# TheJacksonLaboratory/cnn_autoencoder

Measured on AMD Instinct MI355X. Metric: tiles/sec, compress+decompress round trip of 1024x1024x3 histology tiles, higher is better.
Workload: dtype f32 (f16x3 split MFMA: 3 f16 MFMAs per product, fp32 accumulate)

## Files before the change

### cnn_autoencoder_amd/_lib.py

```python
from __future__ import annotations

import ctypes
import os
import subprocess
import threading

import torch

_HERE = os.path.dirname(os.path.abspath(__file__))
LIB_PATH = os.environ.get('CAE_LIB') or os.path.join(_HERE, 'libcae_hip.so')
_lock = threading.Lock()
_lib = None

c_void_p = ctypes.c_void_p
c_int = ctypes.c_int
c_size_t = ctypes.c_size_t
c_float = ctypes.c_float

SYMBOLS = {
    'cae_version': (c_int, []),
    'cae_last_error': (ctypes.c_char_p, []),
    'cae_free': (None, [c_void_p]),
    'cae_model_create': (c_int, [c_int, c_int, c_int, c_int, c_int, ctypes.POINTER(c_void_p)]),
    'cae_model_destroy': (None, [c_void_p]),
# ... 9 lines not shown
    'cae_analysis_levels': (c_int, [c_void_p, c_void_p, c_int, c_int, c_int, c_int, c_void_p, c_void_p, c_void_p]),
    'cae_synthesis': (c_int, [c_void_p, c_void_p, c_int, c_int, c_int, c_void_p, c_int, c_void_p, c_void_p]),
    'cae_model_set_layer_stage': (c_int, [c_void_p, c_int, c_int, c_int, c_void_p, c_void_p, c_void_p, c_void_p, c_int,
                                           c_int, c_int]),
    'cae_model_set_color_layer': (c_int, [c_void_p, c_int, c_int, c_int, c_void_p, c_void_p]),
    'cae_synthesis_multiscale': (c_int, [c_void_p, c_void_p, c_int, c_int, c_int, c_void_p, c_int, c_void_p, c_void_p,
                                          c_void_p]),
    'cae_analysis_symbols': (c_int, [c_void_p, c_void_p, c_int, c_int, c_int, c_int, c_void_p, c_void_p]),
    'cae_synthesis_symbols': (c_int, [c_void_p, c_void_p, c_int, c_int, c_int, c_void_p, c_int, c_void_p]),
    'cae_synthesis_scale': (c_int, [c_void_p, c_void_p, c_int, c_int, c_int, c_int, c_void_p, c_int, c_void_p]),
    'cae_synthesis_symbols_scale': (c_int, [c_void_p, c_void_p, c_int, c_int, c_int, c_int, c_void_p, c_int, c_void_p]),
    'cae_gdn_forward': (c_int, [c_void_p, c_int, c_int, c_void_p, c_int, c_int, c_int, c_void_p, c_void_p]),
    'cae_quantize': (c_int, [c_void_p, c_void_p, c_int, c_int, c_void_p, c_void_p]),
    'cae_quantize_export': (c_int, [c_void_p, c_void_p, c_int, c_int, c_void_p, c_int, c_void_p]),
    'cae_copy_to_host': (c_int, [c_void_p, c_void_p, c_size_t]),
    'cae_dequantize': (c_int, [c_void_p, c_void_p, c_int, c_int, c_void_p, c_void_p]),
    'cae_model_set_density': (c_int, [c_void_p, c_int, c_int, c_void_p, c_void_p, c_void_p, c_void_p, c_float]),
    'cae_model_set_likelihood_form': (c_int, [c_void_p, c_int]),
    'cae_likelihood': (c_int, [c_void_p, c_void_p, c_int, c_int, c_void_p, c_void_p, c_void_p, c_void_p]),
    'cae_tile_ssim': (c_int, [c_void_p, c_void_p, c_int, c_int, c_int, c_int, c_void_p, c_void_p, c_size_t, c_void_p]),
    'cae_tile_delta_e': (c_int, [c_void_p, c_void_p, c_int, c_size_t, c_void_p, c_void_p, c_size_t, c_void_p]),
    'cae_u8hwc_to_planes': (c_int, [c_void_p, c_int, c_int, c_int, c_int, c_void_p, c_void_p]),
    'cae_avgpool2': (c_int, [c_void_p, c_int, c_int, c_int, c_void_p, c_void_p]),
    'cae_msssim_level': (c_int, [c_void_p, c_void_p, c_int, c_int, c_int, c_void_p, c_void_p, c_void_p, c_size_t, c_void_p]),
    'cae_tile_sse': (c_int, [c_void_p, c_void_p, c_int, c_size_t, c_void_p, c_void_p]),
    'cae_model_set_profiling': (c_int, [c_void_p, c_int]),
    'cae_model_get_profile': (c_int, [c_void_p, c_int, c_void_p, c_int, c_void_p, c_int]),
    'cae_t_packed_bytes': (c_size_t, [c_int, c_int, c_int]),
    'cae_t_pack_weights': (c_int, [c_void_p, c_int, c_int, c_int, c_int, c_void_p, c_void_p]),
    'cae_t_from_nchw': (c_int, [c_void_p, c_int, c_int, c_int, c_int, c_int, c_void_p, c_void_p, c_void_p]),
# ... 57 lines not shown
                                     c_void_p, c_void_p]),
    'cae_t_sample_labeled_patches': (c_int, [c_void_p, c_void_p, c_int, c_int, c_int, c_int, c_int, c_void_p, c_void_p,
                                             c_void_p, c_void_p, c_void_p, c_void_p, c_void_p, ctypes.c_uint64,
                                             ctypes.c_uint32, c_float, c_int, c_int, c_int, c_int, c_void_p, c_size_t,
                                             c_void_p, c_void_p, c_void_p]),
    'cae_t_elastic_deform': (c_int, [c_void_p, c_void_p, c_void_p, c_int, c_int, c_int, c_int, c_void_p, c_size_t, c_void_p,
                                     c_void_p, c_void_p]),
    'cae_t_elastic_deform_workspace': (c_size_t, [c_int, c_int, c_int]),
    'cae_cpu_budget': (c_int, []),
    'cae_coder_lockstep': (c_int, []),
    'cae_coder_threads': (c_int, [c_int, c_int]),
    'cae_pmf_to_quantized_cdf': (c_int, [c_void_p, c_int, c_int, c_void_p]),
    'cae_rans_encode_batch': (c_int, [c_void_p, c_void_p, c_int, c_int, c_void_p, c_void_p, c_int]),
    'cae_rans_encode_packed': (c_int, [c_void_p, c_void_p, c_int, c_int, c_void_p, c_void_p, c_int]),
    'cae_rans_decode_batch': (c_int, [c_void_p, c_void_p, c_void_p, c_int, c_int, c_void_p, c_int]),
    'cae_rans_encode_workspace': (c_int, [c_void_p, c_int, c_int, ctypes.POINTER(c_size_t)]),
    'cae_rans_encode_device': (c_int, [c_void_p, c_void_p, c_int, c_int, c_void_p, c_size_t, c_void_p, c_void_p, c_void_p,
                                       c_size_t, c_void_p]),
    'cae_rans_decode_device': (c_int, [c_void_p, c_void_p, c_size_t, c_void_p, c_int, c_int, c_void_p, c_void_p, c_void_p]),
    'cae_door_create': (c_int, [c_void_p, c_void_p, c_int, c_int, ctypes.POINTER(c_void_p)]),
    'cae_door_destroy': (None, [c_void_p]),
    'cae_door_encode': (c_int, [c_void_p, c_void_p, c_int, c_int, c_int, ctypes.POINTER(c_void_p),
                                ctypes.POINTER(c_size_t)]),
    'cae_door_decode_shape': (c_int, [c_void_p, c_void_p, c_size_t, ctypes.POINTER(c_int), ctypes.POINTER(c_int),
                                      ctypes.POINTER(c_int)]),
    'cae_door_decode': (c_int, [c_void_p, c_void_p, c_size_t, c_void_p, c_size_t]),
    'cae_door_stats': (c_int, [c_void_p, c_void_p, c_int, c_int]),
    'cae_door_hold': (c_int, [c_void_p, c_int]),
    'cae_seg_plan': (c_int, [c_void_p, c_void_p, c_int]),
    'cae_seg_workspace_bytes': (c_int, [c_void_p, c_int, c_int, c_int, c_void_p]),
# ... 120 lines not shown
```

### cnn_autoencoder_amd/csrc/cae_copy.cpp

```cpp
#include "cae_hip.h"
#include "cae_internal.hpp"

#include <hsa/hsa.h>
#include <hsa/hsa_ext_amd.h>

#include <mutex>

using namespace cae;

extern "C" int cae_copy_to_host(void *dst_host, const void *src_dev, size_t bytes) {
    if (!dst_host || !src_dev) return fail(CAE_ERR_ARG, "NULL argument");
    if (bytes == 0) return CAE_OK;
    static std::once_flag once;
    static hsa_status_t init_status = HSA_STATUS_SUCCESS;
    std::call_once(once, [] { init_status = hsa_init(); });
    if (init_status != HSA_STATUS_SUCCESS) return fail(CAE_ERR_HIP, "hsa_init failed (%d)", (int)init_status);

    hsa_amd_pointer_info_t si{}, di{};
    si.size = sizeof(si);
    di.size = sizeof(di);
    hsa_status_t st = hsa_amd_pointer_info(const_cast<void *>(src_dev), &si, nullptr, nullptr, nullptr);
    if (st != HSA_STATUS_SUCCESS || si.type != HSA_EXT_POINTER_TYPE_HSA)
        return fail(CAE_ERR_ARG, "source is not a device allocation of this process");
    st = hsa_amd_pointer_info(dst_host, &di, nullptr, nullptr, nullptr);
    if (st != HSA_STATUS_SUCCESS || (di.type != HSA_EXT_POINTER_TYPE_HSA && di.type != HSA_EXT_POINTER_TYPE_LOCKED))
        return fail(CAE_ERR_ARG, "destination must be pinned host memory (hipHostMalloc / a pinned tensor)");
    const char *s0 = (const char *)si.agentBaseAddress, *d0 = (const char *)di.agentBaseAddress;
    if ((const char *)src_dev + bytes > s0 + si.sizeInBytes || (const char *)dst_host + bytes > d0 + di.sizeInBytes)
        return fail(CAE_ERR_ARG, "copy of %zu bytes leaves its allocation", bytes);

    hsa_signal_t sig;
    st = hsa_signal_create(1, 0, nullptr, &sig);
    if (st != HSA_STATUS_SUCCESS) return fail(CAE_ERR_HIP, "hsa_signal_create failed (%d)", (int)st);
    st = hsa_amd_memory_async_copy(dst_host, di.agentOwner, src_dev, si.agentOwner, bytes, 0, nullptr, sig);
    if (st != HSA_STATUS_SUCCESS) {
        hsa_signal_destroy(sig);
        return fail(CAE_ERR_HIP, "hsa_amd_memory_async_copy failed (%d)", (int)st);
    }
    while (hsa_signal_wait_scacquire(sig, HSA_SIGNAL_CONDITION_LT, 1, UINT64_MAX, HSA_WAIT_STATE_BLOCKED) >= 1) {
    }
    hsa_signal_destroy(sig);
    return CAE_OK;
}
```

### cnn_autoencoder_amd/csrc/cae_entropy.cpp

```cpp
#include "cae_hip.h"
#include "cae_internal.hpp"

#include <algorithm>
#include <atomic>
#include <cmath>
#include <cstdio>
#include <cstdlib>
#include <cstring>
#include <mutex>
#include <string>
#include <thread>

#include <sched.h>

namespace cae {

static constexpr uint64_t kRansL = 1ull << 31;
static constexpr uint32_t kPrecision = 16;
static constexpr uint32_t kBypassBits = 4;
static constexpr uint32_t kMaxBypass = (1u << kBypassBits) - 1;
#ifndef CAE_CODER_LOCKSTEP
#define CAE_CODER_LOCKSTEP 2
#endif
static constexpr int kLockMax = 4;
// ... 350 lines not shown
                }
            }
        }
    };
    if (threads == 1) {
        work();
    } else {
        std::vector<std::thread> pool;
        for (int t = 0; t < threads; ++t) pool.emplace_back(work);
        for (auto &t : pool) t.join();
    }
    if (rc.load() != 0) return fail(rc.load(), "%s", first_err.c_str());
    return CAE_OK;
}

}

int rans_encode_chunk(const EntropyTables &T, const int32_t *symbols, int hw, size_t headroom, uint8_t **out,
                      size_t *out_len) {
    const int32_t *sy[1] = {symbols};
    return encode_streams<1>(T, sy, hw, out, out_len, headroom);
}

int rans_encode_chunk_pair(const EntropyTables &T, const int32_t *const *symbols, int hw, size_t headroom, uint8_t **out,
                           size_t *out_len) {
    return encode_streams<2>(T, symbols, hw, out, out_len, headroom);
}

int rans_decode_chunk(const EntropyTables &T, const uint8_t *buf, size_t len, int hw, int32_t *symbols) {
    const uint8_t *b[1] = {buf};
// ... 67 lines not shown
int cae_rans_encode_batch(cae_model_t *mm, const int32_t *symbols, int n_streams, int hw, uint8_t **out_bufs,
                          size_t *out_lens, int threads) {
    Model *m = reinterpret_cast<Model *>(mm);
    if (!m || !symbols || !out_bufs || !out_lens) return fail(CAE_ERR_ARG, "NULL argument");
    if (m->ent.channels == 0) return fail(CAE_ERR_ARG, "entropy model not set");
    if (n_streams < 1 || hw < 0) return fail(CAE_ERR_ARG, "bad shape");
    for (int i = 0; i < n_streams; ++i) {
        out_bufs[i] = nullptr;
        out_lens[i] = 0;
    }
    const EntropyTables &T = m->ent;
    const size_t per = (size_t)T.channels * hw;
    const int lock = lockstep_width();
    const int items = (n_streams + lock - 1) / lock;
    int rc = parallel_streams(items, threads, [&](int it) {
        int i = lock * it;
        const int end = std::min(n_streams, i + lock);
        int r = CAE_OK;
        const int32_t *sy[kLockMax];
        for (; r == CAE_OK && i + 3 < end; i += 4) {
            for (int k = 0; k < 4; ++k) sy[k] = symbols + per * (i + k);
            r = encode_streams<4>(T, sy, hw, &out_bufs[i], &out_lens[i]);
        }
        for (; r == CAE_OK && i + 1 < end; i += 2) {
            sy[0] = symbols + per * i;
            sy[1] = symbols + per * (i + 1);
            r = encode_streams<2>(T, sy, hw, &out_bufs[i], &out_lens[i]);
        }
        if (r == CAE_OK && i < end) {
            sy[0] = symbols + per * i;
            r = encode_streams<1>(T, sy, hw, &out_bufs[i], &out_lens[i]);
        }
        return r;
    });
    if (rc != 0)
        for (int i = 0; i < n_streams; ++i) {
            free(out_bufs[i]);
            out_bufs[i] = nullptr;
        }
    return rc;
}

int cae_rans_encode_packed(cae_model_t *mm, const int32_t *symbols, int n_streams, int hw, uint8_t **out_buf,
                           size_t *offsets, int threads) {
    if (!out_buf || !offsets) return fail(CAE_ERR_ARG, "NULL argument");
    *out_buf = nullptr;
    std::vector<uint8_t *> bufs((size_t)std::max(n_streams, 1), nullptr);
    std::vector<size_t> lens((size_t)std::max(n_streams, 1), 0);
    int rc = cae_rans_encode_batch(mm, symbols, n_streams, hw, bufs.data(), lens.data(), threads);
    if (rc) return rc;
    offsets[0] = 0;
    for (int i = 0; i < n_streams; ++i) offsets[i + 1] = offsets[i] + lens[i];
    uint8_t *packed = (uint8_t *)malloc(offsets[n_streams] ? offsets[n_streams] : 1);
    if (!packed) rc = fail(CAE_ERR_NOMEM, "out of memory (%zu bytes)", offsets[n_streams]);
    if (rc == CAE_OK)
        rc = parallel_streams(n_streams, threads, [&](int i) {
            memcpy(packed + offsets[i], bufs[i], lens[i]);
            return (int)CAE_OK;
        });
    for (int i = 0; i < n_streams; ++i) free(bufs[i]);
    if (rc) {
        free(packed);
        return rc;
    }
    *out_buf = packed;
    return CAE_OK;
}

int cae_rans_decode_batch(cae_model_t *mm, const uint8_t *const *bufs, const size_t *lens, int n_streams, int hw,
                          int32_t *symbols, int threads) {
    Model *m = reinterpret_cast<Model *>(mm);
    if (!m || !symbols || !bufs || !lens) return fail(CAE_ERR_ARG, "NULL argument");
    if (m->ent.channels == 0) return fail(CAE_ERR_ARG, "entropy model not set");
    if (n_streams < 1 || hw < 0) return fail(CAE_ERR_ARG, "bad shape");
    const EntropyTables &T = m->ent;
    const size_t per = (size_t)T.channels * hw;
    const int lock = lockstep_width();
    const int items = (n_streams + lock - 1) / lock;
    return parallel_streams(items, threads, [&](int it) {
        int i = lock * it;
        const int end = std::min(n_streams, i + lock);
        int r = CAE_OK;
        int32_t *sy[kLockMax];
        for (; r == CAE_OK && i + 3 < end; i += 4) {
            for (int k = 0; k < 4; ++k) sy[k] = symbols + per * (i + k);
            r = decode_streams<4>(T, bufs + i, lens + i, hw, sy);
        }
        for (; r == CAE_OK && i + 1 < end; i += 2) {
            sy[0] = symbols + per * i;
            sy[1] = symbols + per * (i + 1);
            r = decode_streams<2>(T, bufs + i, lens + i, hw, sy);
        }
        if (r == CAE_OK && i < end) {
            sy[0] = symbols + per * i;
            r = decode_streams<1>(T, bufs + i, lens + i, hw, sy);
        }
        return r;
    });
}

}
```

### cnn_autoencoder_amd/csrc/cae_internal.hpp

```cpp
#pragma once
#include <cstdarg>
#include <cstddef>
#include <cstdint>
#include <mutex>
#include <utility>
#include <vector>

namespace cae {

int fail(int code, const char *fmt, ...);

void dev_free(void *p);

struct DevBuf {
    void *p = nullptr;
    size_t bytes = 0;
    DevBuf() = default;
    DevBuf(DevBuf &&o) noexcept : p(o.p), bytes(o.bytes) {
        o.p = nullptr;
        o.bytes = 0;
    }
    DevBuf &operator=(DevBuf &&o) noexcept {
        if (this != &o) {
            reset();
// ... 64 lines not shown
    };
    std::vector<EncSym> enc;
    static constexpr int kLutBits = 10;
    std::vector<uint16_t> lut;
    void build_tables();
};

int rans_encode_chunk(const EntropyTables &T, const int32_t *symbols, int hw, size_t headroom, uint8_t **out,
                      size_t *out_len);
int rans_encode_chunk_pair(const EntropyTables &T, const int32_t *const *symbols, int hw, size_t headroom, uint8_t **out,
                           size_t *out_len);
int rans_decode_chunk(const EntropyTables &T, const uint8_t *buf, size_t len, int hw, int32_t *symbols);
int rans_decode_chunk_pair(const EntropyTables &T, const uint8_t *const *bufs, const size_t *lens, int hw,
                           int32_t *const *symbols);

struct DevEntropy {
    DevBuf buf;
    uint64_t version = 0;
    size_t enc = 0, cdf = 0, lut = 0, len = 0, off = 0;
};

struct Model {
    int c_org = 0, c_net = 0, c_bn = 0, L = 0, ks = 3;
    std::vector<Layer> enc, dec;
    EntropyTables ent;
    uint64_t ent_version = 0;
    DevEntropy ent_dev;
    int ensure_ent_device();
    DevBuf medians_dev;
    bool medians_dirty = false;
// ... 30 lines not shown
```

### cnn_autoencoder_amd/entropy.py

```python
from __future__ import annotations

import ctypes
import threading
from typing import List, Optional, Sequence, Tuple

import numpy as np
import torch
import torch.nn as nn
import torch.nn.functional as F

from . import _lib


_SYNC_MU = threading.Lock()


class _LowerBoundFn(torch.autograd.Function):

    @staticmethod
    def forward(ctx, x, bound):
        ctx.save_for_backward(x, bound)
        return torch.max(x, bound)

    @staticmethod
# ... 501 lines not shown
            lens = (ctypes.c_size_t * n)(*[strings.nbytes(i) for i in range(n)])
        else:
            keep = [s if isinstance(s, bytes) else bytes(s) for s in strings]
            bufs = (ctypes.c_char_p * n)(*keep)
            lens = (ctypes.c_size_t * n)(*[len(s) for s in keep])
        if out is None:
            sym = np.empty((n, self.channels, hw), dtype=np.int32)
        else:
            sym = out
            if sym.shape != (n, self.channels, hw) or sym.dtype != np.int32 or not sym.flags.c_contiguous:
                raise ValueError('out must be a C-contiguous int32 array of shape (B,C,hw)')
        _lib.check(_lib.lib().cae_rans_decode_batch(h.ptr, bufs, lens, n, hw, sym.ctypes.data, threads))
        return sym

    @torch.no_grad()
    def encode_symbols_device(self, sym: torch.Tensor) -> PackedStreams:
        h = self._sync_handle()
        if sym.dim() < 2 or sym.size(1) != self.channels:
            raise ValueError(f'Invalid symbol shape {tuple(sym.shape)} for {self.channels} channels')
        packed, offsets = rans_encode_device(h, sym)
        host = packed[:offsets[-1]].cpu().numpy()
        return PackedStreams(host.ctypes.data, offsets, owner=host)

    @torch.no_grad()
    def decode_symbols_device(self, strings: Sequence[bytes], hw: int) -> torch.Tensor:
        return rans_decode_device(self._sync_handle(), self.channels, strings, hw)

    @torch.no_grad()
    def compress(self, x: torch.Tensor, coder: str = 'host') -> List[bytes]:
        if check_coder(coder) == 'device':
# ... 20 lines not shown
```

### cnn_autoencoder_amd/slide.py

```python
from __future__ import annotations

import math
import time
from typing import Dict, List, Sequence, Tuple

import numpy as np
import torch

STATS_WIDTH = 3


def tile_range(rank: int, world: int, n_tiles: int) -> Tuple[int, int]:
    if not (0 <= rank < world) or n_tiles < 0:
        raise ValueError(f'bad partition request rank={rank} world={world} n_tiles={n_tiles}')
    base, rem = divmod(n_tiles, world)
    lo = rank * base + min(rank, rem)
    hi = lo + base + (1 if rank < rem else 0)
    return lo, hi


def tile_stats(nbytes: Sequence[int], sse: Sequence[float], n_samples: int) -> torch.Tensor:
    out = torch.empty((len(nbytes), STATS_WIDTH), dtype=torch.float64)
    out[:, 0] = torch.tensor(list(nbytes), dtype=torch.float64)
    out[:, 1] = torch.tensor(list(sse), dtype=torch.float64)
# ... 60 lines not shown
    sse = float(s[:, 1].sum())
    n = float(s[:, 2].sum())
    n_tiles = s.shape[0]
    mse = sse / max(n, 1.0)
    return dict(tiles=n_tiles, bytes=nbytes, bpp=8.0 * nbytes / max(n_tiles * pixels_per_tile, 1),
                mse=mse, rmse=math.sqrt(mse), psnr=(10.0 * math.log10(255.0 ** 2 / mse) if mse > 0 else float('inf')))


def _dev():
    from . import _lib
    return _lib.require_gpu()


class _PinnedRing:

    def __init__(self, slots: int):
        self.slots = slots
        self._bufs = [None] * slots
        self._readers = [None] * slots

    def take(self, k: int, shape, dtype) -> torch.Tensor:
        i = k % self.slots
        reader, self._readers[i] = self._readers[i], None
        if reader is not None:
            reader.synchronize()
        buf = self._bufs[i]
        if buf is None or buf.shape != tuple(shape) or buf.dtype != dtype:
            buf = self._bufs[i] = torch.empty(tuple(shape), dtype=dtype, pin_memory=True)
        return buf

    def read_by(self, k: int, event) -> None:
        self._readers[k % self.slots] = event


def _clock(tm, key, t0):
    if tm is not None:
        tm[key].append(time.perf_counter() - t0)


class SlideCoder:

    def __init__(self, codec, coder_threads: int = 0, coder: str = 'host'):
        from .codec import _module
        from .entropy import check_coder
        self.codec = codec
        self.coder = check_coder(coder)
        self._coder_streams = None
        self.enc = _module(codec._model['encoder'])
        self.dec = _module(codec._model['decoder'])
        self.eb = _module(codec._model['fact_ent'])
        self.level = len(self.dec.synthesis_track)
        self.coder_threads = coder_threads
        self.encode_threads, self.decode_threads = self._split_budget(coder_threads)
        import os
        self.depth = int(os.environ.get('CAE_PIPELINE_DEPTH', '3'))
        self._rings = {}
        self._copy_stream = None
        self.timers = {}

    @staticmethod
    def _split_budget(requested: int = 0):
        from . import _lib
        import os
        if requested and requested > 0:
            return requested, requested
        if os.environ.get('CAE_ENC_THREADS', '0') != '0' and os.environ.get('CAE_DEC_THREADS', '0') != '0':
            return int(os.environ['CAE_ENC_THREADS']), int(os.environ['CAE_DEC_THREADS'])
        budget = int(_lib.lib().cae_cpu_budget())
        dec = max(1, min(16, budget))
# ... 29 lines not shown
    @torch.no_grad()
    def roundtrip(self, tiles_dev: torch.Tensor) -> Tuple[List[bytes], torch.Tensor, torch.Tensor]:
        n, h, w, c = tiles_dev.shape
        payloads = self.compress(tiles_dev)
        rec = self.decompress(payloads, h, w)
        sse = self.tile_sse(rec, tiles_dev).cpu()
        stats = tile_stats([len(p) + 16 for p in payloads], sse.tolist(), h * w * c)
        return payloads, rec, stats

    def _ring(self, name: str) -> _PinnedRing:
        d = self.depth
        slots = {
            't': 2,
            'a': d + 1,
            'd': d + 2,
            'o': 4,
            's': 3,
            'c': 4,
        }[name]
        ring = self._rings.get(name)
        if ring is None or ring.slots != slots:
            ring = self._rings[name] = _PinnedRing(slots)
        return ring

    def _h2d_stream(self):
        if self._copy_stream is None:
            self._copy_stream = torch.cuda.Stream(_dev())
        return self._copy_stream

    def _coder_stream(self, k):
        if self._coder_streams is None:
            self._coder_streams = [torch.cuda.Stream(_dev()) for _ in range(max(1, self.depth))]
        return self._coder_streams[k % len(self._coder_streams)]

    def _launch_analysis(self, k, t, main):
        sym, guard = self.enc.forward_u8_symbols(t, self.eb, defer=True)
        n, C = sym.size(0), sym.size(1)
# ... 16 lines not shown

    def _pull(self, sym, guard, ready, pin, main, tm):
        from . import _lib
        sym = self._in_range(sym, guard, ready, main)
        t0 = time.perf_counter()
        _lib.check(_lib.lib().cae_copy_to_host(pin.data_ptr(), sym.data_ptr(), sym.numel() * 4))
        _clock(tm, 'd2h_copy', t0)
        return pin

    def _host_encode(self, pulled, packed, tm):
        pin = pulled.result()
        t0 = time.perf_counter()
        payloads = self.eb.encode_symbols(pin.numpy(), self.encode_threads, packed=packed)
        _clock(tm, 'host_encode', t0)
        return payloads

    def _device_encode(self, k, sym, guard, ready, main, tm):
        sym = self._in_range(sym, guard, ready, main)
        t0 = time.perf_counter()
        with torch.cuda.device(sym.device), torch.cuda.stream(self._coder_stream(k)):
            payloads = self.eb.encode_symbols_device(sym)
        _clock(tm, 'host_encode', t0)
        return payloads

    def _encode_async(self, k, t, main, pull_pool, enc_pool, packed, tm=None):
        sym, guard, ready, pin = self._launch_analysis(k, t, main)
        if self.coder == 'device':
            return enc_pool.submit(self._device_encode, k, sym, guard, ready, main, tm)
        pulled = pull_pool.submit(self._pull, sym, guard, ready, pin, main, tm)
        return enc_pool.submit(self._host_encode, pulled, packed, tm)

    def _decode(self, k, payloads, hw, tm=None):
        t0 = time.perf_counter()
        if self.coder == 'device':
            stream = self._coder_stream(k)
            with torch.cuda.device(stream.device), torch.cuda.stream(stream):
                sym = self.eb.decode_symbols_device(payloads, hw)
        else:
            sym = self._ring('d').take(k, (len(payloads), self.eb.channels, hw), torch.int32)
            self.eb.decode_symbols(payloads, hw, self.decode_threads, out=sym.numpy())
        _clock(tm, 'host_decode', t0)
        return sym

    def _launch_synthesis(self, k, sym, lh, lw, main, up, scale=0):
        if self.coder != 'device':
            with torch.cuda.stream(up):
                sym = sym.to(main.device, non_blocking=True)
                copied = torch.cuda.Event(blocking=True)
                copied.record(up)
            self._ring('d').read_by(k, copied)
            main.wait_event(copied)
        sym.record_stream(main)
        return self.dec.forward_symbols_u8(sym.reshape(sym.size(0), self.eb.channels, lh, lw), self.eb, defer=True,
                                           scale=scale)

    def _to_device(self, batch, k, up, main):
        if isinstance(batch, torch.Tensor) and batch.is_cuda:
            return batch
        arr = batch.numpy() if isinstance(batch, torch.Tensor) else np.ascontiguousarray(batch)
        if arr.dtype != np.uint8 or arr.ndim != 4:
# ... 64 lines not shown
            while inflight:
                j, fut = inflight.pop(0)
                yield from emit(j, fut.result())
            while held:
                yield self._in_range(*held.pop(0))
            while outgoing:
                yield outgoing.pop(0).result()

    @torch.no_grad()
    def run(self, batches: Sequence[torch.Tensor], keep_payloads: bool = False):
        from concurrent.futures import ThreadPoolExecutor
        main = torch.cuda.current_stream(batches[0].device)
        copy_up = self._h2d_stream()
        K = len(batches)
        DEPTH = self.depth
        tm = {key: [] for key in ('host_encode', 'host_decode', 'wait_host', 'd2h_copy')}
        all_payloads, stats_parts = [], []
        device = self.coder == 'device'
        n0, h0, w0, _ = batches[0].shape
        lh0, lw0 = self.enc.latent_size(h0, w0)
        for ring in ([] if device else [self._ring('a'), self._ring('d')]):
            for j in range(ring.slots):
                ring.take(j, (n0, self.eb.channels, lh0 * lw0), torch.int32)

        def decode(k, encoded, hw):
            payloads = encoded.result()
            return payloads, self._decode(k, payloads, hw, tm)

        def stage_d(k, payloads, sym):
            t = batches[k]
            n, h, w, c = t.shape
            rec, guard = self._launch_synthesis(k, sym, h // 2 ** self.level, w // 2 ** self.level, main, copy_up)
            sse = self.tile_sse(rec, t)
            got = torch.cuda.Event()
            got.record(main)
            sse_host = self._ring('s').take(k, (n,), torch.float64)
# ... 6 lines not shown
            nbytes = ([payloads.nbytes(i) + 16 for i in range(len(payloads))] if hasattr(payloads, 'nbytes')
                      else [len(p) + 16 for p in payloads])
            return k, sse_host, landed, guard, nbytes, h * w * c

        pending = []

        def finalize(k, sse_pinned, landed, guard, nbytes, samples):
            rec = self._in_range(None, guard, landed, main)
            sse_host = sse_pinned.tolist()
            if rec is not None:
                sse_host = self.tile_sse(rec, batches[k]).cpu().tolist()
            stats_parts.append(tile_stats(nbytes, sse_host, samples))

        workers = DEPTH if device else 1
        with ThreadPoolExecutor(max_workers=1) as pull_pool, ThreadPoolExecutor(max_workers=workers) as enc_pool, \
                ThreadPoolExecutor(max_workers=workers) as dec_pool:
            futs = {}

            def submit(k):
                lh, lw = self.enc.latent_size(*batches[k].shape[1:3])
                encoded = self._encode_async(k, batches[k], main, pull_pool, enc_pool, not keep_payloads, tm)
                futs[k] = dec_pool.submit(decode, k, encoded, lh * lw)

            for k in range(min(DEPTH, K)):
                submit(k)
            for k in range(K):
                if k + DEPTH < K:
                    submit(k + DEPTH)
                t0 = time.perf_counter()
                payloads, sym = futs.pop(k).result()
                _clock(tm, 'wait_host', t0)
                pending.append(stage_d(k, payloads, sym))
                if keep_payloads:
                    all_payloads.append(payloads)
                del payloads
# ... 140 lines not shown
```

### include/cae_hip.h

```cpp
#ifndef CAE_HIP_H
#define CAE_HIP_H

#include <stddef.h>
#include <stdint.h>

#ifdef __cplusplus
extern "C" {
#endif

typedef struct cae_model cae_model_t;

enum cae_status {
    CAE_OK = 0,
    CAE_ERR_ARG = -1,
    CAE_ERR_HIP = -2,
    CAE_ERR_NOMEM = -3,
    CAE_ERR_UNSUPPORTED = -4,
    CAE_ERR_CORRUPT = -5,
    CAE_ERR_RANGE = -6
};

enum cae_track { CAE_ANALYSIS = 0, CAE_SYNTHESIS = 1 };
enum cae_pixfmt {
    CAE_FMT_U8_HWC = 0,
// ... 69 lines not shown
int cae_likelihood(cae_model_t *m, const float *latents_dev, int n, int hw, float *y_hat_dev,
                   float *likelihood_dev, double *bits_dev, void *stream);

int cae_tile_ssim(const uint8_t *a_dev, const uint8_t *b_dev, int n, int h, int w, int c, double *ssim_dev,
                  double *workspace_dev, size_t workspace_elems, void *stream);

int cae_tile_delta_e(const uint8_t *a_dev, const uint8_t *b_dev, int n, size_t pixels, double *delta_dev,
                     double *workspace_dev, size_t workspace_elems, void *stream);

int cae_u8hwc_to_planes(const uint8_t *tiles_dev, int n, int h, int w, int c, float *planes_dev, void *stream);
int cae_avgpool2(const float *in_dev, int planes, int h, int w, float *out_dev, void *stream);
int cae_msssim_level(const float *x_dev, const float *y_dev, int planes, int h, int w, const float *window11_dev,
                     double *ssim_cs_dev, double *workspace_dev, size_t workspace_elems, void *stream);

int cae_copy_to_host(void *dst_pinned_host, const void *src_dev, size_t bytes);

int cae_tile_sse(const uint8_t *a_dev, const uint8_t *b_dev, int n, size_t elems, double *sse_dev, void *stream);

int cae_model_set_profiling(cae_model_t *m, int enable);
int cae_model_get_profile(cae_model_t *m, int track, double *ms, int n_slots, int *calls, int reset);

size_t cae_t_packed_bytes(int contract_channels, int out_channels, int kernel_size);
int cae_t_pack_weights(const float *w_dev, int dim0, int dim1, int kernel_size, int contract_dim, void *packed_dev, void *stream);
int cae_t_from_nchw(const float *x_nchw_dev, int n, int c, int h, int w, int cp, void *out16, float *out32, void *stream);
int cae_t_to_nchw(const float *t32, int n, int c, int h, int w, int cp, float *out_nchw_dev, void *stream);
int cae_t_set_samples_per_block(int npb);
int cae_t_conv_forward(const void *x16, int n, int h, int w, int cin_p, const void *packed, int kernel_size, float *z32,
                       void *z16, int cout_p, const float *bias, void *stream);
int cae_t_conv_dgrad_ext(const void *gz16, int n, int oh, int ow, int cout_p, const void *packed, int kernel_size, int h,
                         int w, float *gext32, int cin_p, void *stream);
// ... 84 lines not shown
                    const float *beta1, const float *beta2, const float *eps, const float *weight_decay,
                    const float *max_norm, const int *step, float *partial_ws, size_t partial_elems, void *stream);

int cae_cpu_budget(void);
int cae_coder_lockstep(void);
int cae_coder_threads(int requested, int n_streams);

int cae_pmf_to_quantized_cdf(const float *pmf_host, int n, int precision, uint32_t *cdf_host );

int cae_rans_encode_batch(cae_model_t *m, const int32_t *symbols_host, int n_streams, int hw,
                          uint8_t **out_bufs, size_t *out_lens, int threads);
int cae_rans_encode_packed(cae_model_t *m, const int32_t *symbols_host, int n_streams, int hw, uint8_t **out_buf,
                           size_t *offsets, int threads);
int cae_rans_decode_batch(cae_model_t *m, const uint8_t *const *bufs, const size_t *lens, int n_streams,
                          int hw, int32_t *symbols_host, int threads);

int cae_rans_encode_workspace(cae_model_t *m, int n_streams, int hw, size_t *bytes);
int cae_rans_encode_device(cae_model_t *m, const int32_t *symbols_dev, int n_streams, int hw, uint8_t *out_dev,
                           size_t out_capacity, int64_t *offsets_dev, int32_t *status_dev, void *workspace_dev,
                           size_t workspace_bytes, void *stream);
int cae_rans_decode_device(cae_model_t *m, const uint8_t *bytes_dev, size_t bytes_len, const int64_t *offsets_dev,
                           int n_streams, int hw, int32_t *symbols_dev, int32_t *status_dev, void *stream);

typedef struct cae_door cae_door_t;
int cae_door_create(cae_model_t *analysis, cae_model_t *synthesis, int max_batch, int inflight, cae_door_t **out);
void cae_door_destroy(cae_door_t *door);
int cae_door_encode(cae_door_t *door, const uint8_t *tile_host, int h, int w, int c, uint8_t **out, size_t *out_len);
int cae_door_decode_shape(cae_door_t *door, const uint8_t *chunk_host, size_t len, int *h, int *w, int *c);
int cae_door_decode(cae_door_t *door, const uint8_t *chunk_host, size_t len, uint8_t *out_host, size_t out_capacity);
enum cae_door_stat {
// ... 91 lines not shown
```

Measured before the change: 4104.

## Fuse host rANS encode/decode round trip into per-item chained DMA pipeline

```diff
diff --git a/cnn_autoencoder_amd/_lib.py b/cnn_autoencoder_amd/_lib.py
--- a/cnn_autoencoder_amd/_lib.py
+++ b/cnn_autoencoder_amd/_lib.py
@@ -47,6 +47,7 @@
     'cae_quantize': (c_int, [c_void_p, c_void_p, c_int, c_int, c_void_p, c_void_p]),
     'cae_quantize_export': (c_int, [c_void_p, c_void_p, c_int, c_int, c_void_p, c_int, c_void_p]),
     'cae_copy_to_host': (c_int, [c_void_p, c_void_p, c_size_t]),
+    'cae_copy_to_device': (c_int, [c_void_p, c_void_p, c_size_t]),
     'cae_dequantize': (c_int, [c_void_p, c_void_p, c_int, c_int, c_void_p, c_void_p]),
     'cae_model_set_density': (c_int, [c_void_p, c_int, c_int, c_void_p, c_void_p, c_void_p, c_void_p, c_float]),
     'cae_model_set_likelihood_form': (c_int, [c_void_p, c_int]),
@@ -134,6 +135,8 @@
     'cae_rans_encode_batch': (c_int, [c_void_p, c_void_p, c_int, c_int, c_void_p, c_void_p, c_int]),
     'cae_rans_encode_packed': (c_int, [c_void_p, c_void_p, c_int, c_int, c_void_p, c_void_p, c_int]),
     'cae_rans_decode_batch': (c_int, [c_void_p, c_void_p, c_void_p, c_int, c_int, c_void_p, c_int]),
+    'cae_rans_roundtrip_packed': (c_int, [c_void_p, c_void_p, c_int, c_int, c_void_p, c_void_p, c_void_p, c_void_p, c_void_p,
+                                          c_int, c_int, c_void_p]),
     'cae_rans_encode_workspace': (c_int, [c_void_p, c_int, c_int, ctypes.POINTER(c_size_t)]),
     'cae_rans_encode_device': (c_int, [c_void_p, c_void_p, c_int, c_int, c_void_p, c_size_t, c_void_p, c_void_p, c_void_p,
                                        c_size_t, c_void_p]),
diff --git a/cnn_autoencoder_amd/csrc/cae_copy.cpp b/cnn_autoencoder_amd/csrc/cae_copy.cpp
--- a/cnn_autoencoder_amd/csrc/cae_copy.cpp
+++ b/cnn_autoencoder_amd/csrc/cae_copy.cpp
@@ -8,31 +8,40 @@
 
 using namespace cae;
 
-extern "C" int cae_copy_to_host(void *dst_host, const void *src_dev, size_t bytes) {
-    if (!dst_host || !src_dev) return fail(CAE_ERR_ARG, "NULL argument");
-    if (bytes == 0) return CAE_OK;
+namespace cae {
+
+int copy_route(void *dst, const void *src, size_t bytes, bool to_device, CopyRoute *route) {
     static std::once_flag once;
     static hsa_status_t init_status = HSA_STATUS_SUCCESS;
     std::call_once(once, [] { init_status = hsa_init(); });
     if (init_status != HSA_STATUS_SUCCESS) return fail(CAE_ERR_HIP, "hsa_init failed (%d)", (int)init_status);
 
-    hsa_amd_pointer_info_t si{}, di{};
-    si.size = sizeof(si);
-    di.size = sizeof(di);
-    hsa_status_t st = hsa_amd_pointer_info(const_cast<void *>(src_dev), &si, nullptr, nullptr, nullptr);
-    if (st != HSA_STATUS_SUCCESS || si.type != HSA_EXT_POINTER_TYPE_HSA)
-        return fail(CAE_ERR_ARG, "source is not a device allocation of this process");
-    st = hsa_amd_pointer_info(dst_host, &di, nullptr, nullptr, nullptr);
-    if (st != HSA_STATUS_SUCCESS || (di.type != HSA_EXT_POINTER_TYPE_HSA && di.type != HSA_EXT_POINTER_TYPE_LOCKED))
-        return fail(CAE_ERR_ARG, "destination must be pinned host memory (hipHostMalloc / a pinned tensor)");
-    const char *s0 = (const char *)si.agentBaseAddress, *d0 = (const char *)di.agentBaseAddress;
-    if ((const char *)src_dev + bytes > s0 + si.sizeInBytes || (const char *)dst_host + bytes > d0 + di.sizeInBytes)
+    void *dev = to_device ? dst : const_cast<void *>(src);
+    void *host = to_device ? const_cast<void *>(src) : dst;
+    hsa_amd_pointer_info_t vi{}, hi{};
+    vi.size = sizeof(vi);
+    hi.size = sizeof(hi);
+    hsa_status_t st = hsa_amd_pointer_info(dev, &vi, nullptr, nullptr, nullptr);
+    if (st != HSA_STATUS_SUCCESS || vi.type != HSA_EXT_POINTER_TYPE_HSA)
+        return fail(CAE_ERR_ARG, "%s is not a device allocation of this process", to_device ? "destination" : "source");
+    st = hsa_amd_pointer_info(host, &hi, nullptr, nullptr, nullptr);
+    if (st != HSA_STATUS_SUCCESS || (hi.type != HSA_EXT_POINTER_TYPE_HSA && hi.type != HSA_EXT_POINTER_TYPE_LOCKED))
+        return fail(CAE_ERR_ARG, "%s must be pinned host memory (hipHostMalloc / a pinned tensor)",
+                    to_device ? "source" : "destination");
+    const char *v0 = (const char *)vi.agentBaseAddress, *h0 = (const char *)hi.agentBaseAddress;
+    if ((const char *)dev + bytes > v0 + vi.sizeInBytes || (const char *)host + bytes > h0 + hi.sizeInBytes)
         return fail(CAE_ERR_ARG, "copy of %zu bytes leaves its allocation", bytes);
+    route->dst_agent = (to_device ? vi : hi).agentOwner.handle;
+    route->src_agent = (to_device ? hi : vi).agentOwner.handle;
+    return CAE_OK;
+}
 
+int copy_slice(const CopyRoute &route, void *dst, const void *src, size_t bytes) {
     hsa_signal_t sig;
-    st = hsa_signal_create(1, 0, nullptr, &sig);
+    hsa_status_t st = hsa_signal_create(1, 0, nullptr, &sig);
     if (st != HSA_STATUS_SUCCESS) return fail(CAE_ERR_HIP, "hsa_signal_create failed (%d)", (int)st);
-    st = hsa_amd_memory_async_copy(dst_host, di.agentOwner, src_dev, si.agentOwner, bytes, 0, nullptr, sig);
+    st = hsa_amd_memory_async_copy(dst, hsa_agent_t{route.dst_agent}, src, hsa_agent_t{route.src_agent}, bytes, 0, nullptr,
+                                   sig);
     if (st != HSA_STATUS_SUCCESS) {
         hsa_signal_destroy(sig);
         return fail(CAE_ERR_HIP, "hsa_amd_memory_async_copy failed (%d)", (int)st);
@@ -42,3 +51,56 @@
     hsa_signal_destroy(sig);
     return CAE_OK;
 }
+
+}
+
+static int copy_whole(void *dst, const void *src, size_t bytes, bool to_device) {
+    if (!dst || !src) return fail(CAE_ERR_ARG, "NULL argument");
+    if (bytes == 0) return CAE_OK;
+    CopyRoute route;
+    if (int rc = copy_route(dst, src, bytes, to_device, &route)) return rc;
+    return copy_slice(route, dst, src, bytes);
+}
+
+static int dma_slice(void *route, void *dst, const void *src, size_t bytes) {
+    return copy_slice(*static_cast<const CopyRoute *>(route), dst, src, bytes);
+}
+
+extern "C" {
+
+int cae_copy_to_host(void *dst_host, const void *src_dev, size_t bytes) { return copy_whole(dst_host, src_dev, bytes, false); }
+
+int cae_copy_to_device(void *dst_dev, const void *src_host, size_t bytes) { return copy_whole(dst_dev, src_host, bytes, true); }
+
+int cae_rans_roundtrip_packed(cae_model_t *mm, const int32_t *symbols_dev, int n_streams, int hw, int32_t *staged_host,
+                              int32_t *decoded_host, int32_t *decoded_dev, uint8_t **out_buf, size_t *offsets, int threads,
+                              int running_cap, double *seconds) {
+    Model *m = reinterpret_cast<Model *>(mm);
+    if (!m || !symbols_dev || !staged_host || !decoded_host || !decoded_dev || !out_buf || !offsets)
+        return fail(CAE_ERR_ARG, "NULL argument");
+    *out_buf = nullptr;
+    if (m->ent.channels == 0) return fail(CAE_ERR_ARG, "entropy model not set");
+    if (n_streams < 1 || hw < 0) return fail(CAE_ERR_ARG, "bad shape");
+    const size_t bytes = (size_t)n_streams * m->ent.channels * hw * sizeof(int32_t);
+    CopyRoute down, up;
+    if (bytes) {
+        if (int rc = copy_route(staged_host, symbols_dev, bytes, false, &down)) return rc;
+        if (int rc = copy_route(decoded_dev, decoded_host, bytes, true, &up)) return rc;
+    }
+    ItemChain ch;
+    ch.src = symbols_dev;
+    ch.staged = staged_host;
+    ch.pull = dma_slice;
+    ch.pull_ctx = &down;
+    ch.decoded = decoded_host;
+    ch.dst = decoded_dev;
+    ch.push = dma_slice;
+    ch.push_ctx = &up;
+    ch.running_cap = running_cap;
+    const int rc = rans_item_chain(m->ent, ch, n_streams, hw, out_buf, offsets, threads);
+    if (seconds)
+        for (int k = 0; k < 4; ++k) seconds[k] = ch.seconds[k];
+    return rc;
+}
+
+}
diff --git a/cnn_autoencoder_amd/csrc/cae_entropy.cpp b/cnn_autoencoder_amd/csrc/cae_entropy.cpp
--- a/cnn_autoencoder_amd/csrc/cae_entropy.cpp
+++ b/cnn_autoencoder_amd/csrc/cae_entropy.cpp
@@ -3,10 +3,13 @@
 
 #include <algorithm>
 #include <atomic>
+#include <chrono>
 #include <cmath>
+#include <condition_variable>
 #include <cstdio>
 #include <cstdlib>
 #include <cstring>
+#include <map>
 #include <mutex>
 #include <string>
 #include <thread>
@@ -388,6 +391,158 @@
     return CAE_OK;
 }
 
+int encode_item(const EntropyTables &T, const int32_t *symbols, size_t per, int i, int end, int hw, uint8_t **out_bufs,
+                size_t *out_lens) {
+    int r = CAE_OK;
+    const int32_t *sy[kLockMax];
+    for (; r == CAE_OK && i + 3 < end; i += 4) {
+        for (int k = 0; k < 4; ++k) sy[k] = symbols + per * (i + k);
+        r = encode_streams<4>(T, sy, hw, &out_bufs[i], &out_lens[i]);
+    }
+    for (; r == CAE_OK && i + 1 < end; i += 2) {
+        sy[0] = symbols + per * i;
+        sy[1] = symbols + per * (i + 1);
+        r = encode_streams<2>(T, sy, hw, &out_bufs[i], &out_lens[i]);
+    }
+    if (r == CAE_OK && i < end) {
+        sy[0] = symbols + per * i;
+        r = encode_streams<1>(T, sy, hw, &out_bufs[i], &out_lens[i]);
+    }
+    return r;
+}
+
+int decode_item(const EntropyTables &T, const uint8_t *const *bufs, const size_t *lens, size_t per, int i, int end, int hw,
+                int32_t *symbols) {
+    int r = CAE_OK;
+    int32_t *sy[kLockMax];
+    for (; r == CAE_OK && i + 3 < end; i += 4) {
+        for (int k = 0; k < 4; ++k) sy[k] = symbols + per * (i + k);
+        r = decode_streams<4>(T, bufs + i, lens + i, hw, sy);
+    }
+    for (; r == CAE_OK && i + 1 < end; i += 2) {
+        sy[0] = symbols + per * i;
+        sy[1] = symbols + per * (i + 1);
+        r = decode_streams<2>(T, bufs + i, lens + i, hw, sy);
+    }
+    if (r == CAE_OK && i < end) {
+        sy[0] = symbols + per * i;
+        r = decode_streams<1>(T, bufs + i, lens + i, hw, sy);
+    }
+    return r;
+}
+
+int pack_streams(uint8_t *const *bufs, const size_t *lens, int n_streams, int threads, uint8_t **out_buf, size_t *offsets) {
+    offsets[0] = 0;
+    for (int i = 0; i < n_streams; ++i) offsets[i + 1] = offsets[i] + lens[i];
+    uint8_t *packed = (uint8_t *)malloc(offsets[n_streams] ? offsets[n_streams] : 1);
+    if (!packed) return fail(CAE_ERR_NOMEM, "out of memory (%zu bytes)", offsets[n_streams]);
+    int rc = parallel_streams(n_streams, threads, [&](int i) {
+        memcpy(packed + offsets[i], bufs[i], lens[i]);
+        return (int)CAE_OK;
+    });
+    if (rc) {
+        free(packed);
+        return rc;
+    }
+    *out_buf = packed;
+    return CAE_OK;
+}
+
+class ItemGate {
+    struct Waiter {
+        std::condition_variable cv;
+        bool go = false;
+    };
+    std::mutex mu;
+    std::multimap<uint64_t, Waiter *> waiting;
+    uint64_t next_ticket = 0;
+    int running = 0;
+
+  public:
+    uint64_t ticket() {
+        std::lock_guard<std::mutex> lk(mu);
+        return next_ticket++;
+    }
+    void enter(uint64_t t, int cap) {
+        std::unique_lock<std::mutex> lk(mu);
+        if (running < cap && (waiting.empty() || t <= waiting.begin()->first)) {
+            ++running;
+            return;
+        }
+        Waiter w;
+        waiting.emplace(t, &w);
+        w.cv.wait(lk, [&] { return w.go; });
+    }
+    void leave(int cap) {
+        std::lock_guard<std::mutex> lk(mu);
+        --running;
+        while (running < cap && !waiting.empty()) {
+            Waiter *w = waiting.begin()->second;
+            waiting.erase(waiting.begin());
+            ++running;
+            w->go = true;
+            w->cv.notify_one();
+        }
+    }
+};
+ItemGate g_gate;
+
+inline double now_seconds() {
+    return std::chrono::duration<double>(std::chrono::steady_clock::now().time_since_epoch()).count();
+}
+
+}
+
+int rans_item_chain(const EntropyTables &T, ItemChain &ch, int n_streams, int hw, uint8_t **out_buf, size_t *offsets,
+                    int threads) {
+    const bool enc = ch.src != nullptr, dec = ch.decoded != nullptr;
+    if (!enc && !dec) return fail(CAE_ERR_ARG, "NULL argument");
+    if (enc && (!ch.staged || !ch.pull || !out_buf || !offsets)) return fail(CAE_ERR_ARG, "NULL argument");
+    if (dec && (!ch.dst || !ch.push || (!enc && (!ch.in_bufs || !ch.in_lens)))) return fail(CAE_ERR_ARG, "NULL argument");
+    if (T.channels == 0) return fail(CAE_ERR_ARG, "entropy model not set");
+    if (n_streams < 1 || hw < 0) return fail(CAE_ERR_ARG, "bad shape");
+    if (enc) *out_buf = nullptr;
+    const size_t per = (size_t)T.channels * hw;
+    const int lock = lockstep_width();
+    const int items = (n_streams + lock - 1) / lock;
+    std::vector<uint8_t *> bufs(enc ? (size_t)n_streams : 0, nullptr);
+    std::vector<size_t> lens(enc ? (size_t)n_streams : 0, 0);
+    std::vector<double> spent((size_t)items * 4, 0.0);
+    const uint64_t ticket = ch.running_cap > 0 ? g_gate.ticket() : 0;
+    int rc = parallel_streams(items, threads, [&](int it) {
+        const int lo = lock * it, hi = std::min(n_streams, lo + lock);
+        const size_t bytes = per * (size_t)(hi - lo) * sizeof(int32_t);
+        double *sp = &spent[(size_t)it * 4];
+        if (ch.running_cap > 0) g_gate.enter(ticket, ch.running_cap);
+        int r = CAE_OK;
+        const uint8_t *const *pb = ch.in_bufs;
+        const size_t *pl = ch.in_lens;
+        if (enc) {
+            double t0 = now_seconds();
+            if (bytes) r = ch.pull(ch.pull_ctx, ch.staged + per * lo, ch.src + per * lo, bytes);
+            sp[0] = now_seconds() - t0;
+            t0 = now_seconds();
+            if (r == CAE_OK) r = encode_item(T, ch.staged, per, lo, hi, hw, bufs.data(), lens.data());
+            sp[1] = now_seconds() - t0;
+            pb = bufs.data();
+            pl = lens.data();
+        }
+        if (dec && r == CAE_OK) {
+            double t0 = now_seconds();
+            r = decode_item(T, pb, pl, per, lo, hi, hw, ch.decoded);
+            sp[2] = now_seconds() - t0;
+            t0 = now_seconds();
+            if (r == CAE_OK && bytes) r = ch.push(ch.push_ctx, ch.dst + per * lo, ch.decoded + per * lo, bytes);
+            sp[3] = now_seconds() - t0;
+        }
+        if (ch.running_cap > 0) g_gate.leave(ch.running_cap);
+        return r;
+    });
+    for (int it = 0; it < items; ++it)
+        for (int k = 0; k < 4; ++k) ch.seconds[k] += spent[(size_t)it * 4 + k];
+    if (rc == CAE_OK && enc) rc = pack_streams(bufs.data(), lens.data(), n_streams, threads, out_buf, offsets);
+    for (auto *b : bufs) free(b);
+    return rc;
 }
 
 int rans_encode_chunk(const EntropyTables &T, const int32_t *symbols, int hw, size_t headroom, uint8_t **out,
@@ -485,24 +640,7 @@
     const int lock = lockstep_width();
     const int items = (n_streams + lock - 1) / lock;
     int rc = parallel_streams(items, threads, [&](int it) {
-        int i = lock * it;
-        const int end = std::min(n_streams, i + lock);
-        int r = CAE_OK;
-        const int32_t *sy[kLockMax];
-        for (; r == CAE_OK && i + 3 < end; i += 4) {
-            for (int k = 0; k < 4; ++k) sy[k] = symbols + per * (i + k);
-            r = encode_streams<4>(T, sy, hw, &out_bufs[i], &out_lens[i]);
-        }
-        for (; r == CAE_OK && i + 1 < end; i += 2) {
-            sy[0] = symbols + per * i;
-            sy[1] = symbols + per * (i + 1);
-            r = encode_streams<2>(T, sy, hw, &out_bufs[i], &out_lens[i]);
-        }
-        if (r == CAE_OK && i < end) {
-            sy[0] = symbols + per * i;
-            r = encode_streams<1>(T, sy, hw, &out_bufs[i], &out_lens[i]);
-        }
-        return r;
+        return encode_item(T, symbols, per, lock * it, std::min(n_streams, lock * it + lock), hw, out_bufs, out_lens);
     });
     if (rc != 0)
         for (int i = 0; i < n_streams; ++i) {
@@ -520,22 +658,9 @@
     std::vector<size_t> lens((size_t)std::max(n_streams, 1), 0);
     int rc = cae_rans_encode_batch(mm, symbols, n_streams, hw, bufs.data(), lens.data(), threads);
     if (rc) return rc;
-    offsets[0] = 0;
-    for (int i = 0; i < n_streams; ++i) offsets[i + 1] = offsets[i] + lens[i];
-    uint8_t *packed = (uint8_t *)malloc(offsets[n_streams] ? offsets[n_streams] : 1);
-    if (!packed) rc = fail(CAE_ERR_NOMEM, "out of memory (%zu bytes)", offsets[n_streams]);
-    if (rc == CAE_OK)
-        rc = parallel_streams(n_streams, threads, [&](int i) {
-            memcpy(packed + offsets[i], bufs[i], lens[i]);
-            return (int)CAE_OK;
-        });
+    rc = pack_streams(bufs.data(), lens.data(), n_streams, threads, out_buf, offsets);
     for (int i = 0; i < n_streams; ++i) free(bufs[i]);
-    if (rc) {
-        free(packed);
-        return rc;
-    }
-    *out_buf = packed;
-    return CAE_OK;
+    return rc;
 }
 
 int cae_rans_decode_batch(cae_model_t *mm, const uint8_t *const *bufs, const size_t *lens, int n_streams, int hw,
@@ -549,24 +674,7 @@
     const int lock = lockstep_width();
     const int items = (n_streams + lock - 1) / lock;
     return parallel_streams(items, threads, [&](int it) {
-        int i = lock * it;
-        const int end = std::min(n_streams, i + lock);
-        int r = CAE_OK;
-        int32_t *sy[kLockMax];
-        for (; r == CAE_OK && i + 3 < end; i += 4) {
-            for (int k = 0; k < 4; ++k) sy[k] = symbols + per * (i + k);
-            r = decode_streams<4>(T, bufs + i, lens + i, hw, sy);
-        }
-        for (; r == CAE_OK && i + 1 < end; i += 2) {
-            sy[0] = symbols + per * i;
-            sy[1] = symbols + per * (i + 1);
-            r = decode_streams<2>(T, bufs + i, lens + i, hw, sy);
-        }
-        if (r == CAE_OK && i < end) {
-            sy[0] = symbols + per * i;
-            r = decode_streams<1>(T, bufs + i, lens + i, hw, sy);
-        }
-        return r;
+        return decode_item(T, bufs, lens, per, lock * it, std::min(n_streams, lock * it + lock), hw, symbols);
     });
 }
 
diff --git a/cnn_autoencoder_amd/csrc/cae_internal.hpp b/cnn_autoencoder_amd/csrc/cae_internal.hpp
--- a/cnn_autoencoder_amd/csrc/cae_internal.hpp
+++ b/cnn_autoencoder_amd/csrc/cae_internal.hpp
@@ -102,6 +102,30 @@
 int rans_decode_chunk_pair(const EntropyTables &T, const uint8_t *const *bufs, const size_t *lens, int hw,
                            int32_t *const *symbols);
 
+using SliceCopy = int (*)(void *ctx, void *dst, const void *src, size_t bytes);
+struct ItemChain {
+    const int32_t *src = nullptr;
+    int32_t *staged = nullptr;
+    SliceCopy pull = nullptr;
+    void *pull_ctx = nullptr;
+    int32_t *decoded = nullptr;
+    int32_t *dst = nullptr;
+    SliceCopy push = nullptr;
+    void *push_ctx = nullptr;
+    const uint8_t *const *in_bufs = nullptr;
+    const size_t *in_lens = nullptr;
+    int running_cap = 0;
+    double seconds[4] = {0, 0, 0, 0};
+};
+int rans_item_chain(const EntropyTables &T, ItemChain &ch, int n_streams, int hw, uint8_t **out_buf, size_t *offsets,
+                    int threads);
+
+struct CopyRoute {
+    uint64_t dst_agent = 0, src_agent = 0;
+};
+int copy_route(void *dst, const void *src, size_t bytes, bool to_device, CopyRoute *route);
+int copy_slice(const CopyRoute &route, void *dst, const void *src, size_t bytes);
+
 struct DevEntropy {
     DevBuf buf;
     uint64_t version = 0;
diff --git a/cnn_autoencoder_amd/entropy.py b/cnn_autoencoder_amd/entropy.py
--- a/cnn_autoencoder_amd/entropy.py
+++ b/cnn_autoencoder_amd/entropy.py
@@ -539,6 +539,28 @@
         return sym
 
     @torch.no_grad()
+    def roundtrip_symbols(self, sym: torch.Tensor, staged: torch.Tensor, decoded: torch.Tensor, out: torch.Tensor,
+                          threads: int = 0, running_cap: int = 0):
+        h = self._sync_handle()
+        n = sym.size(0)
+        hw = sym.numel() // (n * self.channels)
+        if sym.dtype != torch.int32 or not sym.is_cuda or not sym.is_contiguous() or sym.size(1) != self.channels:
+            raise ValueError(f'expected contiguous int32 (B,{self.channels},hw) symbols on the GPU, got {sym.dtype} '
+                             f'{tuple(sym.shape)}')
+        for name, t, cuda in (('staged', staged, False), ('decoded', decoded, False), ('out', out, True)):
+            if (t.dtype != torch.int32 or t.numel() != sym.numel() or not t.is_contiguous() or t.is_cuda != cuda
+                    or not (cuda or t.is_pinned())):
+                raise ValueError(f'{name} must be a contiguous int32 {"device" if cuda else "pinned host"} tensor with one '
+                                 'element per symbol')
+        buf = ctypes.c_void_p()
+        offs = (ctypes.c_size_t * (n + 1))()
+        seconds = (ctypes.c_double * 4)()
+        _lib.check(_lib.lib().cae_rans_roundtrip_packed(h.ptr, sym.data_ptr(), n, hw, staged.data_ptr(), decoded.data_ptr(),
+                                                        out.data_ptr(), ctypes.byref(buf), offs, threads, running_cap,
+                                                        seconds))
+        return PackedStreams(buf.value, list(offs)), list(seconds)
+
+    @torch.no_grad()
     def encode_symbols_device(self, sym: torch.Tensor) -> PackedStreams:
         h = self._sync_handle()
         if sym.dim() < 2 or sym.size(1) != self.channels:
diff --git a/cnn_autoencoder_amd/slide.py b/cnn_autoencoder_amd/slide.py
--- a/cnn_autoencoder_amd/slide.py
+++ b/cnn_autoencoder_amd/slide.py
@@ -98,8 +98,9 @@
 
 class _PinnedRing:
 
-    def __init__(self, slots: int):
+    def __init__(self, slots: int, device=None):
         self.slots = slots
+        self.device = device
         self._bufs = [None] * slots
         self._readers = [None] * slots
 
@@ -110,7 +111,11 @@
             reader.synchronize()
         buf = self._bufs[i]
         if buf is None or buf.shape != tuple(shape) or buf.dtype != dtype:
-            buf = self._bufs[i] = torch.empty(tuple(shape), dtype=dtype, pin_memory=True)
+            if self.device is None:
+                buf = torch.empty(tuple(shape), dtype=dtype, pin_memory=True)
+            else:
+                buf = torch.empty(tuple(shape), dtype=dtype, device=self.device)
+            self._bufs[i] = buf
         return buf
 
     def read_by(self, k: int, event) -> None:
@@ -137,6 +142,10 @@
         self.coder_threads = coder_threads
         self.encode_threads, self.decode_threads = self._split_budget(coder_threads)
         import os
+        from . import _lib
+        self.item_threads = int(os.environ.get('CAE_ITEM_THREADS', '0')) or (
+            coder_threads if coder_threads and coder_threads > 0
+            else max(1, min(self.encode_threads + self.decode_threads, int(_lib.lib().cae_cpu_budget()))))
         self.depth = int(os.environ.get('CAE_PIPELINE_DEPTH', '3'))
         self._rings = {}
         self._copy_stream = None
@@ -196,13 +205,14 @@
             't': 2,
             'a': d + 1,
             'd': d + 2,
+            'u': d + 3,
             'o': 4,
             's': 3,
             'c': 4,
         }[name]
         ring = self._rings.get(name)
         if ring is None or ring.slots != slots:
-            ring = self._rings[name] = _PinnedRing(slots)
+            ring = self._rings[name] = _PinnedRing(slots, device=_dev() if name == 'u' else None)
         return ring
 
     def _h2d_stream(self):
@@ -249,6 +259,15 @@
         payloads = self.eb.encode_symbols(pin.numpy(), self.encode_threads, packed=packed)
         _clock(tm, 'host_encode', t0)
         return payloads
+
+    def _host_roundtrip(self, ranged, pin, back, out, as_list, tm):
+        sym = ranged.result()
+        payloads, spent = self.eb.roundtrip_symbols(sym.reshape(sym.size(0), sym.size(1), -1), pin, back, out,
+                                                    self.item_threads, self.item_threads)
+        if tm is not None:
+            for key, s in zip(('d2h_copy', 'host_encode', 'host_decode', 'h2d_copy'), spent):
+                tm[key].append(s)
+        return (list(payloads) if as_list else payloads), out
 
     def _device_encode(self, k, sym, guard, ready, main, tm):
         sym = self._in_range(sym, guard, ready, main)
@@ -278,7 +297,7 @@
         return sym
 
     def _launch_synthesis(self, k, sym, lh, lw, main, up, scale=0):
-        if self.coder != 'device':
+        if not sym.is_cuda:
             with torch.cuda.stream(up):
                 sym = sym.to(main.device, non_blocking=True)
                 copied = torch.cuda.Event(blocking=True)
@@ -373,12 +392,12 @@
         copy_up = self._h2d_stream()
         K = len(batches)
         DEPTH = self.depth
-        tm = {key: [] for key in ('host_encode', 'host_decode', 'wait_host', 'd2h_copy')}
+        tm = {key: [] for key in ('host_encode', 'host_decode', 'wait_host', 'd2h_copy', 'h2d_copy')}
         all_payloads, stats_parts = [], []
         device = self.coder == 'device'
         n0, h0, w0, _ = batches[0].shape
         lh0, lw0 = self.enc.latent_size(h0, w0)
-        for ring in ([] if device else [self._ring('a'), self._ring('d')]):
+        for ring in ([] if device else [self._ring('a'), self._ring('d'), self._ring('u')]):
             for j in range(ring.slots):
                 ring.take(j, (n0, self.eb.channels, lh0 * lw0), torch.int32)
 
@@ -415,11 +434,20 @@
 
         workers = DEPTH if device else 1
         with ThreadPoolExecutor(max_workers=1) as pull_pool, ThreadPoolExecutor(max_workers=workers) as enc_pool, \
-                ThreadPoolExecutor(max_workers=workers) as dec_pool:
+                ThreadPoolExecutor(max_workers=workers) as dec_pool, \
+                ThreadPoolExecutor(max_workers=min(DEPTH + 1, 3)) as host_pool:
             futs = {}
 
             def submit(k):
                 lh, lw = self.enc.latent_size(*batches[k].shape[1:3])
+                if not device:
+                    shape = (batches[k].shape[0], self.eb.channels, lh * lw)
+                    out = self._ring('u').take(k, shape, torch.int32)
+                    back = self._ring('d').take(k, shape, torch.int32)
+                    sym, guard, ready, pin = self._launch_analysis(k, batches[k], main)
+                    ranged = pull_pool.submit(self._in_range, sym, guard, ready, main)
+                    futs[k] = host_pool.submit(self._host_roundtrip, ranged, pin, back, out, keep_payloads, tm)
+                    return
                 encoded = self._encode_async(k, batches[k], main, pull_pool, enc_pool, not keep_payloads, tm)
                 futs[k] = dec_pool.submit(decode, k, encoded, lh * lw)
 
diff --git a/include/cae_hip.h b/include/cae_hip.h
--- a/include/cae_hip.h
+++ b/include/cae_hip.h
@@ -107,6 +107,7 @@
                      double *ssim_cs_dev, double *workspace_dev, size_t workspace_elems, void *stream);
 
 int cae_copy_to_host(void *dst_pinned_host, const void *src_dev, size_t bytes);
+int cae_copy_to_device(void *dst_dev, const void *src_pinned_host, size_t bytes);
 
 int cae_tile_sse(const uint8_t *a_dev, const uint8_t *b_dev, int n, size_t elems, double *sse_dev, void *stream);
 
@@ -221,6 +222,9 @@
                            size_t *offsets, int threads);
 int cae_rans_decode_batch(cae_model_t *m, const uint8_t *const *bufs, const size_t *lens, int n_streams,
                           int hw, int32_t *symbols_host, int threads);
+int cae_rans_roundtrip_packed(cae_model_t *m, const int32_t *symbols_dev, int n_streams, int hw, int32_t *staged_pinned,
+                              int32_t *decoded_pinned, int32_t *decoded_dev, uint8_t **out_buf, size_t *offsets,
+                              int threads, int running_cap, double *seconds);
 
 int cae_rans_encode_workspace(cae_model_t *m, int n_streams, int hw, size_t *bytes);
 int cae_rans_encode_device(cae_model_t *m, const int32_t *symbols_dev, int n_streams, int hw, uint8_t *out_dev,
```

New measurement: 4123, median of 6. No clear change (+0.4%).
